# lxd99/TPNet

Measured on AMD Instinct MI355X. Metric: temporal edges/sec (proj-update + pairwise readout), higher is better.
Workload: dtype f32; 1 GPU; C2: Wikipedia-shape d=128 B=1000, L=3, synthetic S(8227,1000,E,span) stream of 2399000 edges, decoder-level unit (2 readouts + update per edge); batch=1000, dim=128, num_layer=3, nodes=9228, parallelism=single GPU

## Files before the change

tpnet_amd/csrc/api.hip:

```cpp
#include "tpnet_common.h"

#include <cstring>

namespace tpnet {
thread_local int g_last_hip_error = 0;

int check_state(const tpnet_state* st) {
    if (!st || !st->p0 || !st->q || !st->meta || !st->err) return TPNET_ERR_BAD_ARG;
    if (st->N < 1 || st->d < 1 || st->L < 1 || st->L > TPNET_MAX_LAYERS) return TPNET_ERR_BAD_ARG;
    if (st->N >= (1ll << 31)) return TPNET_ERR_BAD_ARG;
    return TPNET_OK;
}

template <class F> static int64_t most_that_fit(int64_t hi, F fits) {
    int64_t lo = 0;
    while (hi - lo > 1) {
        const int64_t mid = (lo + hi) / 2;
        if (fits(mid)) lo = mid; else hi = mid;
    }
    return lo;
}

static int64_t max_chunk(size_t ws_bytes, int64_t E, int64_t batch) {
    const int64_t hard = ((int64_t)1 << 30) / batch * batch;
// ... 123 lines not shown
};

static int run_stream_windowed(const StreamCall& c, int64_t chunk, int Kmax, size_t region) {
    const tpnet_state& st = c.st;
    const int64_t E = c.E, batch = c.batch;
    hipStream_t s = c.s;
    uint32_t lid = c.launch_id_base;
    const bool have_readout = c.out_pos || c.out_neg;
    char* const arena = reinterpret_cast<char*>((reinterpret_cast<size_t>(c.ws) + 255) / 256 * 256);
    const int64_t n_chunks = (E + chunk - 1) / chunk;
    float* const shared_log = region ? reinterpret_cast<float*>(arena + (size_t)n_chunks * region) : nullptr;
    PlanReplay tag(c, n_chunks == 1 || region, 1, true, window_batches_for(((E < chunk ? E : chunk) + batch - 1) / batch, Kmax),
                   c.flags & ~(uint32_t)TPNET_FLAG_SCHED_WINDOWED, have_readout, chunk, region);
    bool all_kept = true;
    for (int64_t c0 = 0, ci = 0; c0 < E; c0 += chunk, ++lid, ++ci) {
        const int64_t Ec = (E - c0 < chunk) ? (E - c0) : chunk;
        const int64_t nb = (Ec + batch - 1) / batch;
        const int K = window_batches_for(nb, Kmax);
        WPlan p{};
        int rc = region ? wplan_carve(arena + (size_t)ci * region, region, Ec, batch, st.N, st.d, st.L, K, &p, shared_log)
                        : wplan_carve(c.ws, c.ws_bytes, Ec, batch, st.N, st.d, st.L, K, &p);
        if (rc) return rc;
        const WPlanner planner = choose_wplanner(st, &p, Ec, batch, K, c.flags);
        all_kept &= planner.replayable;
        const StreamArgs a = c.args_at(c0);
        const WPlanArgs pa{a.src, a.dst, a.neg, a.t, Ec, batch, c.now_time, c0 > 0 ? c.t + c0 - 1 : nullptr, c.lambda, have_readout,
                           tag.replay};
        rc = planner.build(st, p, pa, s);
        if (rc) return rc;
        const int64_t nw = (Ec + p.Ew - 1) / p.Ew;
        const int64_t nsteps = nw + (have_readout ? st.L : st.L - 1);
        const bool timed = c.timer && c.timer->begin(s);
        for (int64_t j = 0; j < nsteps; ++j) {
            rc = launch_wstep(st, a, p, j, Ec, batch, c.lambda, c.flags, s);
            if (rc) return rc;
        }
        if (timed) c.timer->end(s, nsteps, Ec);
        rc = planner.writeback(st, p, Ec, batch, lid, s, -1);
        if (rc) return rc;
    }
    tag.commit(all_kept);
    return TPNET_OK;
}

static int run_stream_impl(const StreamCall& c) {
    const tpnet_state& st = c.st;
    const int64_t E = c.E, batch = c.batch;
    const double lambda = c.lambda;
    const uint32_t flags = c.flags;
    hipStream_t s = c.s;
    if (E == 0) return TPNET_OK;
    int Kw = 0;
    size_t region = 0;
    const int64_t wchunk = window_chunk(st, c.ws_bytes, E, batch, flags, &Kw, c.tag ? &region : nullptr);
    if (wchunk > 0) return run_stream_windowed(c, wchunk, Kw, region);
    const int64_t chunk = max_chunk(c.ws_bytes, E, batch);
    PlanReplay tag(c, chunk >= E, 2, false, 0, flags, c.out_pos != nullptr, chunk, 0);
    if (chunk < 1) return TPNET_ERR_WORKSPACE;
    uint32_t lid = c.launch_id_base;
    for (int64_t c0 = 0; c0 < E; c0 += chunk) {
        const int64_t Ec = (E - c0 < chunk) ? (E - c0) : chunk;
        Plan p{};
        int rc = plan_carve(c.ws, c.ws_bytes, Ec, batch, &p);
        if (rc) return rc;
        static const int fuse_env = TPNET_DEV_INT(FUSE, -1);
        static const int role_mask = TPNET_DEV_INT(ROLE_MASK, 3);
        const bool fuse = c.out_pos && p.fuse_src && role_mask == 3 &&
                          !(flags & (TPNET_FLAG_EAGER_DECAY | TPNET_FLAG_SEQUENTIAL)) &&
                          (fuse_env >= 0 ? fuse_env == 1 : batch > 1024);
        const StreamArgs a = c.args_at(c0);
        if (!tag.replay) {
            rc = plan_build(st, p, a.src, a.dst, a.t, Ec, batch, c.now_time, c0 > 0 ? c.t + c0 - 1 : nullptr, lambda,
// ... 408 lines not shown
```

tpnet_amd/csrc/plan.hip:

```cpp
#include "tpnet_common.h"

#include <cstdlib>
#include <cstring>
#include <rocprim/block/block_radix_sort.hpp>
#include <rocprim/device/device_radix_sort.hpp>
#include <rocprim/device/device_segmented_radix_sort.hpp>
#include <rocprim/iterator/counting_iterator.hpp>
#include <rocprim/iterator/transform_iterator.hpp>

#ifdef TPNET_STAMPS
#define PSTAMP(slot)                                                                          \
    do {                                                                                      \
        if (dbg && blockIdx.x == 0 && threadIdx.x == 0) {                                     \
            dbg[(slot) * 2 + 0] = __builtin_amdgcn_s_memtime();                               \
            dbg[(slot) * 2 + 1] = __builtin_amdgcn_s_memrealtime();                           \
        }                                                                                     \
    } while (0)
#else
#define PSTAMP(slot) do { } while (0)
#endif

namespace tpnet {

static constexpr uint32_t HEAVY_THRESHOLD = 8u;
// ... 802 lines not shown
                           node_bits, lambda, thr, fuse, st.err);
    TPNET_HIP_TRY(hipGetLastError());
    return TPNET_OK;
}


int wplan_window_batches(int64_t batch, int d, int L) {
    static const char* env = TPNET_DEV_STR(WINDOW);
    (void)L;
    if (d % 4 != 0 || d < 4 || batch < 1) return 0;
    if (batch > 4096) return 0;
    int64_t K = 24576 / batch;
    if (env) K = atoi(env);
    if (K > WIN_MAX_BATCHES) K = WIN_MAX_BATCHES;
    return K >= 2 ? (int)K : 0;
}

int window_batches_for(int64_t nb, int Kmax) {
    static const int fixed = TPNET_DEV_INT(WINDOW_FIXED, 0);
    if (fixed > 0) return fixed < Kmax ? fixed : Kmax;
    static const int num = TPNET_DEV_INT(WINDOW_SQ, 5);
    int K = 2;
    while (K < Kmax && (int64_t)K * K < (int64_t)num * nb) ++K;
    const int64_t nw0 = (nb + K - 1) / K;
    return (int)((nb + nw0 - 1) / nw0);
}

WPlanner choose_wplanner(const tpnet_state& st, const WPlan* p, int64_t Ec, int64_t batch, int K, uint32_t flags) {
    static const int no3 = TPNET_DEV_INT(NO_PLAN3, 0);
    static const int max3 = TPNET_DEV_INT(PLAN3_MAX_BATCHES, 1 << 30);
    const bool small = batch <= PLAN_ONE_MAX;
    if (!(flags & (TPNET_FLAG_PLAN_SORTED | TPNET_FLAG_PLAN_HASHED)) &&
        (p ? wplan_dense_applies(st, *p, Ec, batch, K) : small && wplan_dense_eligible(st.N, st.d, st.L, batch)))
        return {wplan_dense_build, wplan_dense_writeback, true, 256};
    if (!(flags & TPNET_FLAG_PLAN_SORTED) &&
        (p ? !no3 && (Ec + batch - 1) / batch <= max3 && wplan3_applies(st, Ec, batch, K) : small))
        return {wplan3_build, wplan3_writeback, true, WIN_MAX_WINDOWS};
    return {wplan_build, launch_wwriteback, false, 0};
}

bool wplan_medium_chains(int d) {
    static const int off = TPNET_DEV_INT(NO_MEDIUM, 0);
    if (off || d % 4 != 0) return false;
    const Geom g = pick_geom(d);
    return g.w == 4 && d == g.lpp * g.vpl * 4;
}

uint32_t wplan_heavy_threshold(int K, int64_t batch, int d) {
    static const int env = TPNET_DEV_INT(WIN_HEAVY, 0);
    if (env > 0) return (uint32_t)env;
    if (wplan_medium_chains(d)) return 128u;
    const int64_t t = (int64_t)K * batch * d / 24576;
    return (uint32_t)(t < 16 ? 16 : (t > 96 ? 96 : t));
}

int64_t wplan_max_chunk_edges(int64_t batch, int d, int L) {
    static const char* env = TPNET_DEV_STR(WIN_CHUNK_MB);
    const int64_t log_cap = (env ? (int64_t)atoi(env) : 16384) << 20;
    int64_t e = log_cap / (2 * (int64_t)L * d * 4);
    const int64_t hard = (int64_t)(WREF_SLOT_MASK >> 1);
    if (e > hard) e = hard;
    if (e > 65535 * batch) e = 65535 * batch;
    e = e / batch * batch;
    return e < batch ? batch : e;
}

static size_t wplan_extra_bytes(int64_t Ec, int64_t batch, int64_t N, int d, int L, int K) {
    const size_t nc = 2 * (size_t)Ec;
    (void)K;
    const size_t nw = (size_t)((Ec + batch - 1) / batch);
    size_t tot = 0;
// ... 445 lines not shown
```

tpnet_amd/csrc/tpnet_common.h:

```cpp
#pragma once
#include <hip/hip_runtime.h>
#include <stdint.h>
#include <stdlib.h>
#include <new>
#include "../../include/tpnet_hip.h"
#include "tpnet_dev.h"
#include "event_set.hpp"

#ifdef TPNET_DEV
static inline int tpnet_dev_env_int(const char* name, int dflt) { const char* v = getenv(name); return v ? atoi(v) : dflt; }
#define TPNET_DEV_INT(NAME, DFLT) tpnet_dev_env_int("TPNET_DEV_" #NAME, (DFLT))
#define TPNET_DEV_STR(NAME) getenv("TPNET_DEV_" #NAME)
#else
#define TPNET_DEV_INT(NAME, DFLT) (DFLT)
#define TPNET_DEV_STR(NAME) ((const char*)nullptr)
#endif

namespace tpnet {

struct NodeMeta {
    uint32_t ver;
    uint32_t pad0;
    double tref[2];
    uint64_t pad1;
// ... 240 lines not shown
                float* shared_log = nullptr, bool shard = false);
size_t wplan_bytes_shard(int64_t max_edges, int64_t batch, int64_t N, int d, int L);
size_t wplan_log_bytes(int64_t max_edges, int d, int L);
struct WPlanArgs {
    const int64_t *src, *dst, *neg;
    const double* t;
    int64_t Ec, batch;
    double now_time;
    const double* t_prev_dev;
    double lambda;
    bool want_readout;
    bool replay;
    int64_t own = -1;
    uint32_t* status = nullptr;
};
int wplan_build(const tpnet_state& st, const WPlan& p, const WPlanArgs& a, hipStream_t s);
int wplan3_build(const tpnet_state& st, const WPlan& p, const WPlanArgs& a, hipStream_t s);
int wplan_dense_build(const tpnet_state& st, const WPlan& p, const WPlanArgs& a, hipStream_t s);
int launch_wwriteback(const tpnet_state& st, const WPlan& p, int64_t Ec, int64_t batch, uint32_t launch_id, hipStream_t s, int64_t own = -1);
int wplan3_writeback(const tpnet_state& st, const WPlan& p, int64_t Ec, int64_t batch, uint32_t launch_id, hipStream_t s, int64_t own = -1);
int wplan_dense_writeback(const tpnet_state& st, const WPlan& p, int64_t Ec, int64_t batch, uint32_t launch_id, hipStream_t s, int64_t own = -1);
bool wplan3_applies(const tpnet_state& st, int64_t Ec, int64_t batch, int K);
size_t wplan3_table_bytes(int64_t Ec, int64_t batch);
size_t wplan3_blk_bytes(int64_t Ec, int64_t batch);
bool wplan_dense_eligible(int64_t N, int d, int L, int64_t batch);
size_t wplan_dense_bytes(int64_t Ec, int64_t batch, int64_t N, int d, int L);
bool wplan_dense_applies(const tpnet_state& st, const WPlan& p, int64_t Ec, int64_t batch, int K);
bool wplan_dense_applies_shard(const tpnet_state& st, const WPlan& p, int64_t Ec, int64_t batch, int K);

struct WPlanner {
    decltype(&wplan_build) build;
    decltype(&launch_wwriteback) writeback;
    bool replayable;
    int max_windows;
};
WPlanner choose_wplanner(const tpnet_state& st, const WPlan* p, int64_t Ec, int64_t batch, int K, uint32_t flags);
uint32_t wplan_heavy_threshold(int K, int64_t batch, int d);
bool wplan_medium_chains(int d);
int launch_wstep(const tpnet_state& st, const StreamArgs& a, const WPlan& p, int64_t j, int64_t Ec, int64_t batch,
                 double lambda, uint32_t flags, hipStream_t s);
int check_state(const tpnet_state* st);

extern thread_local int g_last_hip_error;
#define TPNET_HIP_TRY(expr)                                   \
    do {                                                      \
        hipError_t _e = (expr);                               \
        if (_e != hipSuccess) {                               \
            tpnet::g_last_hip_error = (int)_e;                \
            return TPNET_ERR_HIP;                             \
        }                                                     \
    } while (0)
#define TPNET_CATCH_BAD_ALLOC \
    catch (const std::bad_alloc&) { tpnet::g_last_hip_error = (int)hipErrorOutOfMemory; return TPNET_ERR_HIP; }

}
```

tpnet_amd/csrc/wshard.hip:

```cpp
#include "wplan_dense.hpp"

#include <rocprim/device/device_radix_sort.hpp>
#include <rocprim/device/device_scan.hpp>
#include <rocprim/iterator/counting_iterator.hpp>
#include <rocprim/iterator/transform_iterator.hpp>

#include <dlfcn.h>
#include <cstring>
#include <memory>
#include <vector>

namespace tpnet {

struct WsRccl {
    int (*send)(const void*, size_t, int, int, void*, hipStream_t) = nullptr;
    int (*recv)(void*, size_t, int, int, void*, hipStream_t) = nullptr;
    int (*group_start)() = nullptr;
    int (*group_end)() = nullptr;
};
bool rows_rccl_api(WsRccl* out);

static constexpr int WS_MAXG = 64;
static constexpr int kWsFloat32 = 7;

// ... 555 lines not shown
    if (phases & WS_PH_EXCHANGE) {
        WsRccl api;
        if (!comm || !rows_rccl_api(&api)) return TPNET_ERR_BAD_ARG;
        const size_t d = (size_t)w->st.d, Ld = (size_t)w->st.L * d;
        float* halo_p0 = w->st.p0 + (size_t)w->n_owned * d;
        float* halo_q = w->st.q + (size_t)w->n_owned * Ld;
        int bad = api.group_start();
        for (int r = 0; r < G; ++r) {
            if (r == me) continue;
            if (mine) {
                bad |= api.send(w->send_p0, (size_t)mine * d, kWsFloat32, r, comm, s);
                bad |= api.send(w->send_q, (size_t)mine * Ld, kWsFloat32, r, comm, s);
            }
            if (w->chunk_cnt[r]) {
                bad |= api.recv(halo_p0 + (size_t)w->hstart[r] * d, (size_t)w->chunk_cnt[r] * d, kWsFloat32, r, comm, s);
                bad |= api.recv(halo_q + (size_t)w->hstart[r] * Ld, (size_t)w->chunk_cnt[r] * Ld, kWsFloat32, r, comm, s);
            }
        }
        bad |= api.group_end();
        if (bad) return TPNET_ERR_HIP;
    }
    return TPNET_OK;
}

int tpnet_wshard_step(tpnet_wshard* w, void* comm, int64_t j, uint32_t phases, float* out_pos, float* out_neg, void* stream) {
    if (!w || j < 0 || j >= w->nsteps) return TPNET_ERR_BAD_ARG;
    hipStream_t s = (hipStream_t)stream;
    const int G = w->G, me = w->me, d = w->st.d, L = w->st.L;
    if (phases & WS_PH_LAUNCH) {
        StreamArgs a = w->a;
        a.out_pos = out_pos;
        a.out_neg = out_neg;
        if ((out_pos || out_neg) != w->have_readout) return TPNET_ERR_BAD_ARG;
        int rc = launch_wstep(w->st, a, w->p, j, w->E, w->batch, w->lambda, w->flags, s);
        if (rc) return rc;
    }
    if (G == 1) return TPNET_OK;
    const int64_t ns = w->send_base[j + 1] - w->send_base[j], nr = w->recv_base[j + 1] - w->recv_base[j];
    if ((phases & WS_PH_PACK) && ns > 0) {
        if (!w->sendbuf) return TPNET_ERR_BAD_ARG;
        int g = (int)((ns + 15) / 16);
        if (g > 4096) g = 4096;
        hipLaunchKernelGGL((k_ws_copy<true>), dim3(g), dim3(256), 0, s, w->ent[1] + w->send_base[j], (uint32_t)ns, w->p.log, w->sendbuf, L, d);
    }
    if ((phases & WS_PH_EXCHANGE) && (ns > 0 || nr > 0)) {
        WsRccl api;
        if (!comm || !rows_rccl_api(&api)) return TPNET_ERR_BAD_ARG;
        int bad = api.group_start();
        size_t so = 0, ro = 0;
        for (int r = 0; r < G; ++r) {
            const size_t cs = (size_t)w->send_cnt[(size_t)j * G + r], cr = (size_t)w->recv_cnt[(size_t)j * G + r];
            if (r != me && cs) bad |= api.send(w->sendbuf + so * d, cs * d, kWsFloat32, r, comm, s);
            if (r != me && cr) bad |= api.recv(w->recvbuf + ro * d, cr * d, kWsFloat32, r, comm, s);
            so += cs;
            ro += cr;
        }
        bad |= api.group_end();
        if (bad) return TPNET_ERR_HIP;
    }
    if ((phases & WS_PH_UNPACK) && nr > 0) {
        if (!w->recvbuf) return TPNET_ERR_BAD_ARG;
        int g = (int)((nr + 15) / 16);
        if (g > 4096) g = 4096;
        hipLaunchKernelGGL((k_ws_copy<false>), dim3(g), dim3(256), 0, s, w->ent[0] + w->recv_base[j], (uint32_t)nr, w->p.log, w->recvbuf, L, d);
    }
    TPNET_HIP_TRY(hipGetLastError());
    return TPNET_OK;
// ... 57 lines not shown
```

tpnet_amd/csrc/wstep.hip:

```cpp
#include "readout.hpp"

namespace tpnet {

static constexpr int WB = 256;
#ifndef TPNET_WPIPE_MINW
#define TPNET_WPIPE_MINW 4
#endif
constexpr int wpipe_min_waves(int lpp, int vpl, int l, bool full) {
    return (lpp <= 32 && vpl == 1) ? TPNET_WPIPE_MINW
         : (lpp == 32 && vpl == 2) ? ((full && l <= 3) ? 3 : 2)
         : (lpp == 64 && vpl == 1) ? (full ? 3 : 2)
         : 2;
}

__device__ __forceinline__ float pow_rep(float g, int n) {
    float r = 1.0f;
    for (int z = 0; z < n; ++z) r *= g;
    return r;
}

__device__ __forceinline__ const float* partner_row(const tpnet_state& S, const WPlan& P, int layer, int32_t pv,
                                                    uint32_t ref, float g, float& gp) {
    const int d = S.d, L = S.L;
    if (layer == 1) {
        gp = 1.0f;
        return S.p0 + (int64_t)pv * d;
    }
    gp = pow_rep(g, layer - 1);
    if (ref & WREF_TABLE) return S.q + (((int64_t)(ref & 1u) * S.N + pv) * L + (layer - 2)) * (int64_t)d;
    return P.log + ((int64_t)(ref & WREF_SLOT_MASK) * L + (layer - 2)) * (int64_t)d;
}

__device__ __forceinline__ const float* chain_start(const tpnet_state& S, const WPlan& P, const Chain& c, int layer,
                                                    float& g0) {
    const int d = S.d, L = S.L;
    g0 = pow_rep(c.g_first, layer);
    if (c.prev_ref & WREF_TABLE)
        return S.q + (((int64_t)(c.prev_ref & 1u) * S.N + c.target) * L + (layer - 1)) * (int64_t)d;
    return P.log + ((int64_t)(c.prev_ref & WREF_SLOT_MASK) * L + (layer - 1)) * (int64_t)d;
}

template <int LPP, int VPL, bool FULL>
__device__ __forceinline__ void chain_light(const tpnet_state& S, const WPlan& P, Chain c, bool valid, int layer,
                                            double lambda, int gl, unsigned long long* dbg) {
    (void)dbg;
    STAMP(5);
    constexpr int W = 4, F = VPL * W, U = (F == 4) ? 8 : 4;
    const int d = S.d, L = S.L;
    const int nvec = d / W;
    if (!valid) { c.cnt = 0; c.target = 0; c.j0 = 0; c.prev_ref = WREF_TABLE; c.g_first = 1.0f; }
    float g0;
    const float* qold = chain_start(S, P, c, layer, g0);
    const bool from_table = (c.prev_ref & WREF_TABLE) != 0;
    const int32_t* __restrict__ s_partner = P.base.s_partner;
    const float* __restrict__ s_coef = P.base.s_coef;

    for (int c0 = 0; c0 < (FULL ? 1 : nvec); c0 += LPP * VPL) {
        float acc[F], sblk[F], srun[F];
#pragma unroll
        for (int j = 0; j < VPL; ++j) {
            const int vi = c0 + j * LPP + gl;
            ldv_maybe<W, FULL>(qold, vi, valid && vi < nvec, &acc[j * W]);
        }
#pragma unroll
        for (int x = 0; x < F; ++x) { sblk[x] = 0.0f; srun[x] = 0.0f; }
        bool firstblk = false;
        float cur_dec = 1.0f;
        int32_t nx_pv = 0;
        float nx_w = 0.0f, nx_glog = 1.0f, nx_decr = 1.0f;
        uint32_t nx_ref = 0u;
        auto fetch_meta = [&](uint32_t r0) {
            const uint32_t jm = c.j0 + r0 + (uint32_t)gl;
            const bool mine = r0 + (uint32_t)gl < c.cnt;
            nx_pv = mine ? s_partner[jm] : 0;
            nx_w = mine ? s_coef[jm] : 0.0f;
            nx_ref = mine ? P.s_ref[jm] : 0u;
            nx_glog = mine ? P.s_g[jm] : 1.0f;
            nx_decr = mine ? P.s_dec[jm] : 1.0f;
        };
        fetch_meta(0u);
        for (uint32_t r0 = 0; __any(r0 < c.cnt); r0 += LPP) {
            const int32_t my_pv = nx_pv;
            const float my_w = nx_w;
            const uint32_t my_ref = nx_ref;
            const float my_glog = nx_glog;
            const float my_dec = pow_rep(nx_decr, layer);
// ... 39 lines not shown
                        }
                        if (fl & WREF_BLK_TAIL) {
#pragma unroll
                            for (int x = 0; x < F; ++x) srun[x] = firstblk ? sblk[x] : srun[x] + sblk[x];
                            firstblk = false;
                        }
                        if (fl & WREF_RUN_TAIL) {
#pragma unroll
                            for (int x = 0; x < F; ++x) {
                                acc[x] *= cur_dec;
                                acc[x] = acc[x] + srun[x];
                            }
                            float* lrow = P.log + ((int64_t)pos * L + (layer - 1)) * (int64_t)d;
#pragma unroll
                            for (int j = 0; j < VPL; ++j) {
                                const int vi = c0 + j * LPP + gl;
                                if (FULL || vi < nvec) stv<W>(lrow, vi, &acc[j * W]);
                            }
                        }
                    }
                }
            };
            if (__any(n_here > 0u)) issue(0u, rA);
            for (uint32_t k0 = 0; __any(k0 < n_here); k0 += 2 * US) {
                const bool more1 = __any(k0 + US < n_here);
                if (more1) issue(k0 + US, rB);
                consume(k0, rA);
                if (more1) {
                    if (__any(k0 + 2 * US < n_here)) issue(k0 + 2 * US, rA);
                    consume(k0 + US, rB);
                }
            }
        }
    }
    STAMP(6);
}

struct HRec {
    uint32_t row;
    float w, gp;
};
static_assert(sizeof(HRec) == 12, "HRec must be 12 bytes");

__device__ __forceinline__ uint32_t partner_row_index(const tpnet_state& S, int layer, int32_t pv, uint32_t ref, float g, float& gp,
                                                      bool& in_log) {
    const int L = S.L;
    in_log = false;
    if (layer == 1) {
        gp = 1.0f;
        return (uint32_t)pv;
    }
    gp = pow_rep(g, layer - 1);
    if (ref & WREF_TABLE) return (uint32_t)((((int64_t)(ref & 1u) * S.N + pv) * L) + (layer - 2));
    in_log = true;
    return (uint32_t)((int64_t)(ref & WREF_SLOT_MASK) * L + (layer - 2));
}

template <int LPH>
struct HeavyCfg {
    static constexpr int G = WB / LPH;
    static constexpr int PW = LPH * 4;
    static constexpr int TSEG = 128 * (8 * 4 + PW + 2) / (8 * 3 + PW + 2);
    static constexpr int HT = (TSEG + G - 1) / G < 4 ? (TSEG + G - 1) / G : 4;
    static constexpr int O_START = 0, O_END = 64, O_DECP = 128 , O_TOFF = 192 ,
                         O_RLIST = 260 , O_NRUN = 324, O_RTOFF = 328 , O_RSLOT = 396 ,
                         O_RSUM = 460 , O_REC = O_RSUM + 64 * PW ,
                         O_PART = O_REC + TSEG * WIN_BLOCK * 3 , O_TPOS = O_PART + TSEG * PW ,
                         O_TN = O_TPOS + TSEG , WORDS = O_TN + TSEG;
};

template <int LPH>
__device__ __forceinline__ void chain_heavy(const tpnet_state& S, const WPlan& P, const Chain c, int part, int layer,
                                            double lambda, uint32_t b0 ,
                                            uint32_t* __restrict__ lds_u, unsigned long long* dbg) {
    (void)dbg;
    STAMP(0);
    using H = HeavyCfg<LPH>;
    constexpr int G = H::G, PW = H::PW, TSEG = H::TSEG, HT = H::HT;
    const int tid = threadIdx.x, g = tid / LPH, gl = tid % LPH;
    const int d = S.d, L = S.L;
    const int nvec = d / 4;
    const int vi = part * LPH + gl;
    const bool vok = vi < nvec;
    uint32_t* run_start = lds_u + H::O_START;
    uint32_t* run_end = lds_u + H::O_END;
    float* r_decp = reinterpret_cast<float*>(lds_u + H::O_DECP);
    uint32_t* task_off = lds_u + H::O_TOFF;
    uint32_t* rlist = lds_u + H::O_RLIST;
    uint32_t* nrun_p = lds_u + H::O_NRUN;
    uint32_t* r_toff = lds_u + H::O_RTOFF;
    uint32_t* r_slot = lds_u + H::O_RSLOT;
    float* r_sum = reinterpret_cast<float*>(lds_u + H::O_RSUM);
    HRec* rec = reinterpret_cast<HRec*>(lds_u + H::O_REC);
    float* lds_part = reinterpret_cast<float*>(lds_u + H::O_PART);
    uint32_t* t_pos = lds_u + H::O_TPOS;
    uint32_t* t_n = lds_u + H::O_TN;

    __syncthreads();
    if (tid < 64) { run_start[tid] = 0xFFFFFFFFu; run_end[tid] = 0u; r_decp[tid] = 1.0f; }
    __syncthreads();
    float* dec_bw = r_sum;
    for (uint32_t p0 = 0; p0 < c.cnt; p0 += 8 * WB) {
        uint32_t ref[8], bcq[8];
        float dec[8];
#pragma unroll
        for (int q = 0; q < 8; ++q) {
            const uint32_t p = p0 + (uint32_t)(q * WB + tid);
            const bool in = p < c.cnt;
            ref[q] = in ? P.s_ref[c.j0 + p] : 0u;
            dec[q] = in ? P.s_dec[c.j0 + p] : 1.0f;
            bcq[q] = in ? (uint32_t)P.s_bc[c.j0 + p] : b0;
        }
#pragma unroll
        for (int q = 0; q < 8; ++q) {
            const uint32_t p = p0 + (uint32_t)(q * WB + tid);
            const uint32_t bw = (bcq[q] - b0) & 63u;
            if (ref[q] & WREF_RUN_HEAD) { run_start[bw] = p; dec_bw[bw] = dec[q]; }
            if (ref[q] & WREF_RUN_TAIL) run_end[bw] = p;
        }
    }
    __syncthreads();
    if (tid < 64) {
        const uint32_t st = run_start[tid];
        const bool has = st != 0xFFFFFFFFu;
        const uint32_t nt = has ? (run_end[tid] - st + WIN_BLOCK) / WIN_BLOCK : 0u;
        uint32_t inc = nt;
#pragma unroll
        for (int o = 1; o < 64; o <<= 1) {
            const uint32_t v = (uint32_t)__shfl_up((int)inc, o, 64);
// ... 157 lines not shown
                for (int q = 0; q < 4; ++q) {
                    const uint32_t rr = r0 + q;
                    if (rr < last) {
#pragma unroll
                        for (int x = 0; x < 4; ++x) {
                            acc[x] *= dec[q];
                            acc[x] = acc[x] + rs[q][x];
                        }
                        float* rs_ = r_sum + (size_t)rr * PW + gl * 4;
#pragma unroll
                        for (int x = 0; x < 4; ++x) rs_[x] = acc[x];
                    }
                }
            }
            if (tid == 0) nrun_p[1] = last;
        }
        __syncthreads();
        {
            const uint32_t lastb_ = nrun_p[1];
            for (uint32_t rr = next_run_all + (uint32_t)g; rr < lastb_; rr += G) {
                float v[4];
                const float* rs_ = r_sum + (size_t)rr * PW + gl * 4;
#pragma unroll
                for (int x = 0; x < 4; ++x) v[x] = rs_[x];
                if (vok) {
                    float* lrow = P.log + ((int64_t)r_slot[rr] * L + (layer - 1)) * (int64_t)d;
                    stv<4>(lrow, vi, v);
                }
            }
            next_run_all = lastb_;
        }
        if (tid < 64) next_run = last;
        __syncthreads();
    }
    STAMP(4);
#ifdef TPNET_STAMPS
    if (dbg && (threadIdx.x & 63) == 0) {
        const size_t wv = ((size_t)blockIdx.x * (blockDim.x >> 6) + (threadIdx.x >> 6));
        if (wv < 4000) dbg[(wv * 8 + 7) * 2 + 0] = c.cnt;
    }
#endif
}

template <int LPP, int VPL, int LWORDS>
struct MedCfg {
    static constexpr int GPB = WB / LPP;
    static constexpr int PG = GPB * 16 <= WB ? 16 : WB / GPB;
    static constexpr int SEGP = GPB * PG;
    static constexpr int RW = LPP * VPL * 4;
    static constexpr int O_ROW = 0, O_W = 2 * SEGP, O_GP = 3 * SEGP, O_FL = 4 * SEGP, O_DEC = 5 * SEGP, O_BLK = 6 * SEGP,
                         O_BFL = 7 * SEGP, BCAP_ = (LWORDS - 7 * SEGP - (GPB + 1) - 16 - 4) / (RW + 3),
                         BCAP = BCAP_ > SEGP ? SEGP : BCAP_, O_BDEC = O_BFL + BCAP, O_BSLOT = O_BDEC + BCAP,
                         O_OWN = O_BSLOT + BCAP, O_MISC = O_OWN + GPB + 1, O_SUM = (O_MISC + 16 + 3) / 4 * 4,
                         WORDS = O_SUM + BCAP * RW;
    static_assert(WORDS <= LWORDS, "chain_medium: LDS layout");
    static_assert(BCAP >= 8, "chain_medium: LDS for at least 8 block sums");
};

template <int LPP, int VPL, int LWORDS>
__device__ __forceinline__ void chain_medium(const tpnet_state& S, const WPlan& P, const Chain c, int layer,
                                             uint32_t* __restrict__ lds_u) {
    using M = MedCfg<LPP, VPL, LWORDS>;
    constexpr int W = 4, F = VPL * W, U = (F == 4) ? 8 : 4;
    constexpr int GPB = M::GPB, SEGP = M::SEGP, BCAP = M::BCAP, RW = M::RW;
    static_assert(SEGP <= WB, "a thread per position");
    const int tid = threadIdx.x, g = tid / LPP, gl = tid % LPP;
    const int d = S.d, L = S.L;
    const float** p_row = reinterpret_cast<const float**>(lds_u + M::O_ROW);
    float* p_w = reinterpret_cast<float*>(lds_u + M::O_W);
    float* p_gp = reinterpret_cast<float*>(lds_u + M::O_GP);
    uint32_t* p_fl = lds_u + M::O_FL;
    float* p_dec = reinterpret_cast<float*>(lds_u + M::O_DEC);
    uint32_t* p_blk = lds_u + M::O_BLK;
    uint32_t* b_fl = lds_u + M::O_BFL;
    float* b_dec = reinterpret_cast<float*>(lds_u + M::O_BDEC);
    uint32_t* b_slot = lds_u + M::O_BSLOT;
    uint32_t* own = lds_u + M::O_OWN;
    uint32_t* misc = lds_u + M::O_MISC;
    float* bsum = reinterpret_cast<float*>(lds_u + M::O_SUM);

    float g0;
    const float* qold = chain_start(S, P, c, layer, g0);
    const bool from_table = (c.prev_ref & WREF_TABLE) != 0;
    float acc[F], srun[F];
#pragma unroll
    for (int j = 0; j < VPL; ++j) ldv<W>(g == 0 ? qold : S.p0, j * LPP + gl, &acc[j * W]);
#pragma unroll
    for (int x = 0; x < F; ++x) srun[x] = 0.0f;
    bool firstblk = false;
    float cur_dec = 1.0f;

    for (uint32_t s0 = 0; s0 < c.cnt;) {
        __syncthreads();
        const uint32_t left = c.cnt - s0 < (uint32_t)SEGP ? c.cnt - s0 : (uint32_t)SEGP;
        const uint32_t pg = (left + GPB - 1) / GPB < 2u ? 2u : (left + GPB - 1) / GPB;
        const uint32_t pos = s0 + (uint32_t)tid;
        const bool in = tid < SEGP && pos < c.cnt;
        const uint32_t jm = c.j0 + (in ? pos : 0u);
        const int32_t pv = in ? P.base.s_partner[jm] : 0;
        const float wgt = in ? P.base.s_coef[jm] : 0.0f;
        const uint32_t ref = in ? P.s_ref[jm] : 0u;
        const float glog = in ? P.s_g[jm] : 1.0f;
        const float decr = in ? P.s_dec[jm] : 1.0f;
        if (tid <= GPB) own[tid] = SEGP;
        const bool head = in && (ref & WREF_BLK_HEAD) != 0;
        const unsigned long long hm = __ballot(head);
        const int lane = tid & 63, wave = tid >> 6;
        if (lane == 0 && wave < 4) misc[2 + wave] = (uint32_t)__popcll(hm);
        __syncthreads();
        uint32_t blk = (uint32_t)__popcll(hm & ((2ull << lane) - 1ull)) - 1u;
        for (int wv = 0; wv < wave && wv < 4; ++wv) blk += misc[2 + wv];
        const bool keep = in && blk < (uint32_t)BCAP;
        if (tid < SEGP) {
            float gp;
            const float* row = partner_row(S, P, layer, pv, ref, glog, gp);
            p_row[tid] = row;
// ... 73 lines not shown
                    sb[j * W] = v4.x; sb[j * W + 1] = v4.y; sb[j * W + 2] = v4.z; sb[j * W + 3] = v4.w;
                }
                if (bf & 1u) { firstblk = true; cur_dec = b_dec[b]; }
#pragma unroll
                for (int x = 0; x < F; ++x) srun[x] = firstblk ? sb[x] : srun[x] + sb[x];
                firstblk = false;
                if (bf & 2u) {
#pragma unroll
                    for (int x = 0; x < F; ++x) {
                        acc[x] *= cur_dec;
                        acc[x] = acc[x] + srun[x];
                    }
#pragma unroll
                    for (int j = 0; j < VPL; ++j)
                        slot[j * LPP + gl] = make_float4(acc[j * W], acc[j * W + 1], acc[j * W + 2], acc[j * W + 3]);
                }
            }
        }
        __syncthreads();
        for (uint32_t b = (uint32_t)g; b < nblk; b += GPB) {
            if (b_fl[b] & 2u) {
                const float4* slot = reinterpret_cast<const float4*>(bsum + (size_t)b * RW);
                float* lrow = P.log + ((int64_t)b_slot[b] * L + (layer - 1)) * (int64_t)d;
#pragma unroll
                for (int j = 0; j < VPL; ++j) {
                    const float4 v4 = slot[j * LPP + gl];
                    const float v[4] = {v4.x, v4.y, v4.z, v4.w};
                    stv<W>(lrow, j * LPP + gl, v);
                }
            }
        }
        s0 += npos;
    }
}

constexpr int heavy_lph(int lpp, int vpl) { return lpp * vpl <= 32 ? 4 : (lpp * vpl <= 64 ? 8 : 16); }

struct WStep {
    int64_t w_upd[TPNET_MAX_LAYERS];
    int64_t w_read;
    uint32_t seg[2 * TPNET_MAX_LAYERS + 3];
    int32_t CP;
    int32_t dbg_layer;
    int32_t dbg_skip;
    uint32_t n_active;
    uint32_t hub_ext;
    uint32_t hub_blocks;
    uint32_t med;
};

__device__ __forceinline__ uint32_t big_chains(const WStep& st, const WinDesc& wd, uint32_t n_hub) {
    const uint32_t n = st.med == 3u ? wd.n_med : st.med == 2u ? wd.n_ext : st.med == 1u ? wd.n_ext1 : 0u;
    return n > n_hub ? n : n_hub;
}

__device__ __forceinline__ uint32_t hub_chains(const WStep& st, const WinDesc& wd) {
    if (st.hub_ext == 2 && wd.n_ext * (uint32_t)st.CP <= st.hub_blocks) return wd.n_ext;
    if (st.hub_ext >= 1 && wd.n_ext1 * (uint32_t)st.CP <= st.hub_blocks) return wd.n_ext1;
    return wd.n_heavy;
}

template <int LPP, int VPL, int L, bool FULL, bool RS, bool SHARD = false>
__global__ __launch_bounds__(WB, wpipe_min_waves(LPP, VPL, L, FULL)) void k_wpipe(tpnet_state S, WPlan P, StreamArgs a, WStep st, int64_t Ec, int64_t B,
                                              double lambda, uint32_t flags) {
    constexpr int W = 4;
    constexpr int LPH = heavy_lph(LPP, VPL);
    constexpr int RLPP = RS ? 16 : LPP, RVPL = RS ? 2 : VPL;
    static_assert(!RS || (LPP == 32 && VPL == 1), "readout split: chains on 32 x 1");
    using C = GramCfg<RLPP, L>;
    constexpr bool LR = false;
    constexpr int RWORDS = (RLPP < 16) ? C::NG * (WB / RLPP) : 1;
    constexpr int LWORDS = HeavyCfg<LPH>::WORDS > RWORDS ? HeavyCfg<LPH>::WORDS : RWORDS;
    constexpr int SL = 2 * L;
    __shared__ __attribute__((aligned(16))) uint32_t lds_u[LWORDS];
    const int gl = threadIdx.x % LPP;
    const int g = threadIdx.x / LPP;
    constexpr int GPB = WB / LPP;
    const uint32_t bx = blockIdx.x;
    int sidx = 0;
    uint32_t seg_lo = 0, seg_hi = st.seg[1];
    int64_t w = st.w_upd[0];
#pragma unroll
// ... 72 lines not shown
                const float gs_e = P.e_g[(int64_t)which[s] * Ec + e];
                const uint32_t ref = idok ? ref_e : WREF_TABLE;
                const float gs = idok ? gs_e : 1.0f;
                const float* qb = (ref & WREF_TABLE) ? S.q + ((int64_t)(ref & 1u) * S.N + ids[s]) * ((int64_t)L * d)
                                                     : P.log + (int64_t)(ref & WREF_SLOT_MASK) * ((int64_t)L * d);
                rowp[s * NR] = S.p0 + ids[s] * (int64_t)d;
                rs[s * NR] = 1.0f;
                float gg = 1.0f;
#pragma unroll
                for (int i = 1; i <= L; ++i) {
                    gg *= gs;
                    rowp[s * NR + i] = qb + (int64_t)(i - 1) * d;
                    rs[s * NR + i] = gg;
                }
            }
            if (packed)
                gram_rows<RLPP, RVPL, W, L, FULL, true, LR>(rowp, rs, d, valid, idok, do_scale, out, rgl, stage);
            else
                gram_rows<RLPP, RVPL, W, L, FULL, false, LR>(rowp, rs, d, valid, idok, do_scale, out, rgl, stage);
        }
        BEND();
        return;
    }
    const WinDesc wd = P.wdesc[w];
    unsigned long long* dbg = (st.dbg_layer == layer) ? P.base.dbg : nullptr;
    (void)dbg;
    if (sidx < L) {
#ifdef TPNET_DEV
        if (st.dbg_skip & 1) return;
#endif
        const Chain* __restrict__ heavy = P.chains + wd.start;
        const uint32_t units = hub_chains(st, wd) * (uint32_t)st.CP;
        for (uint32_t h = rb; h < units; h += nblk)
            chain_heavy<LPH>(S, P, heavy[h / (uint32_t)st.CP], (int)(h % (uint32_t)st.CP), layer, lambda,
                             (uint32_t)(w * P.K), lds_u, dbg);
        BEND();
        return;
    }
    if (sidx < SL) {
        if constexpr (FULL) {
            const uint32_t n_hub = hub_chains(st, wd);
            const uint32_t n_big = big_chains(st, wd, n_hub);
            const Chain* __restrict__ list = P.chains + wd.start;
            for (uint32_t m = n_hub + rb; m < n_big; m += nblk) chain_medium<LPP, VPL, LWORDS>(S, P, list[m], layer, lds_u);
        }
        BEND();
        return;
    }
#ifdef TPNET_DEV
    if (st.dbg_skip & 2) return;
#endif
    const uint32_t n_hub = big_chains(st, wd, hub_chains(st, wd));
    const Chain* __restrict__ small = P.chains + wd.start + n_hub;
    const int64_t n_small = (int64_t)wd.n_chains - (int64_t)n_hub;
    for (int64_t base = (int64_t)rb * GPB; base < n_small; base += (int64_t)nblk * GPB) {
        const int64_t idx = base + g;
        const bool valid = idx < n_small;
        const Chain c = small[valid ? idx : 0];
        chain_light<LPP, VPL, FULL>(S, P, c, valid, layer, lambda, gl, dbg);
    }
    BEND();
}

static constexpr int WBS = 256;
__global__ __launch_bounds__(WB) void k_wwriteback(tpnet_state S, WPlan P, int64_t nc, uint32_t bid) {
    const int per = S.L * S.d;
    NodeMeta* meta = reinterpret_cast<NodeMeta*>(S.meta);
    __shared__ uint32_t n_list;
    __shared__ uint32_t l_pos[WBS];
    __shared__ int32_t l_node[WBS];
    __shared__ int32_t l_copy[WBS];
    for (int64_t j0 = (int64_t)blockIdx.x * WBS; j0 < nc; j0 += (int64_t)gridDim.x * WBS) {
        __syncthreads();
        if (threadIdx.x == 0) n_list = 0;
        __syncthreads();
        const int64_t j = j0 + threadIdx.x;
        if (threadIdx.x < WBS && j < nc && (P.s_ref[j] & WREF_LAST_RUN)) {
            const int32_t u = P.base.s_target[j];
            const int c = (int)(meta[u].ver & 1u);
            const uint32_t k = atomicAdd(&n_list, 1u);
            l_pos[k] = (uint32_t)j;
            l_node[k] = u;
            l_copy[k] = c;
        }
        __syncthreads();
        const uint32_t n = n_list;
        if ((per & 3) == 0) {
            const uint32_t pv = (uint32_t)per / 4;
            const uint32_t tot = n * pv;
            for (uint32_t x0 = threadIdx.x; x0 < tot; x0 += 4 * WB) {
                const uint32_t xa = x0, xb = x0 + WB, xc = x0 + 2 * WB, xd = x0 + 3 * WB;
                const uint32_t ka = xa / pv, kb = (xb < tot ? xb : xa) / pv, kc = (xc < tot ? xc : xa) / pv, kd = (xd < tot ? xd : xa) / pv;
// ... 2 lines not shown
                const float4 va = reinterpret_cast<const float4*>(P.log + (int64_t)l_pos[ka] * per)[oa];
                const float4 vb = reinterpret_cast<const float4*>(P.log + (int64_t)l_pos[kb] * per)[ob];
                const float4 vc = reinterpret_cast<const float4*>(P.log + (int64_t)l_pos[kc] * per)[oc];
                const float4 vd = reinterpret_cast<const float4*>(P.log + (int64_t)l_pos[kd] * per)[od];
                reinterpret_cast<float4*>(S.q + ((int64_t)(l_copy[ka] ^ 1) * S.N + l_node[ka]) * (int64_t)per)[oa] = va;
                if (xb < tot) reinterpret_cast<float4*>(S.q + ((int64_t)(l_copy[kb] ^ 1) * S.N + l_node[kb]) * (int64_t)per)[ob] = vb;
                if (xc < tot) reinterpret_cast<float4*>(S.q + ((int64_t)(l_copy[kc] ^ 1) * S.N + l_node[kc]) * (int64_t)per)[oc] = vc;
                if (xd < tot) reinterpret_cast<float4*>(S.q + ((int64_t)(l_copy[kd] ^ 1) * S.N + l_node[kd]) * (int64_t)per)[od] = vd;
            }
        } else {
            for (uint32_t x = threadIdx.x; x < n * (uint32_t)per; x += WB) {
                const uint32_t k = x / (uint32_t)per, o = x - k * (uint32_t)per;
                S.q[((int64_t)(l_copy[k] ^ 1) * S.N + l_node[k]) * (int64_t)per + o] = P.log[(int64_t)l_pos[k] * per + o];
            }
        }
        if (threadIdx.x < n) {
            const uint32_t k = threadIdx.x;
            publish_meta(meta + l_node[k], l_copy[k] ^ 1, P.base.desc[P.s_bc[l_pos[k]]].t_last, bid);
        }
    }
}

int launch_wwriteback(const tpnet_state& st, const WPlan& p, int64_t Ec, int64_t, uint32_t launch_id, hipStream_t s, int64_t) {
    const int64_t nc = 2 * Ec;
    int64_t grid = (nc + WBS - 1) / WBS;
    if (grid > 16384) grid = 16384;
    if (grid < 1) grid = 1;
    hipLaunchKernelGGL(k_wwriteback, dim3((unsigned)grid), dim3(WB), 0, s, st, p, nc, launch_id);
    TPNET_HIP_TRY(hipGetLastError());
    return TPNET_OK;
}

int launch_wstep(const tpnet_state& st, const StreamArgs& a, const WPlan& p, int64_t j, int64_t Ec, int64_t batch,
                 double lambda, uint32_t flags, hipStream_t s) {
    if ((reinterpret_cast<uintptr_t>(a.out_pos) | reinterpret_cast<uintptr_t>(a.out_neg)) & 15) return TPNET_ERR_BAD_ARG;
    if (st.d % 4 != 0) return TPNET_ERR_BAD_ARG;
    const int L = st.L;
    const int64_t nw = (Ec + p.Ew - 1) / p.Ew;
    static const int hb_env = TPNET_DEV_INT(WIN_HB, 0);
    static const int stamp_layer = TPNET_DEV_INT(STAMP_LAYER, 0);
    static const int geo_env = TPNET_DEV_INT(WIN_GEOM, 0);
    const Geom geo = pick_geom(st.d, geo_env == 1);
    const int lph = heavy_lph(geo.lpp, geo.vpl);
    const int GPB = WB / geo.lpp;
    static const int rs_env = TPNET_DEV_INT(WIN_RSPLIT, 1);
    const bool rsplit = rs_env == 1 && geo.lpp == 32 && geo.vpl == 1 && st.d / 4 > 16;
    WStep ws;
    ws.CP = (st.d / 4 + lph - 1) / lph;
    static const int stamp_step = TPNET_DEV_INT(STAMP_STEP, -1);
    ws.dbg_layer = (stamp_layer == -1 && stamp_step >= 0 && j != stamp_step) ? 0 : stamp_layer;
    static const int skip_env = TPNET_DEV_INT(WIN_SKIP, 0);
    ws.dbg_skip = skip_env;
    const bool have_readout = a.out_pos || a.out_neg;
    auto win_edges = [&](int64_t w) { const int64_t e0 = w * p.Ew; return (Ec - e0 < p.Ew) ? Ec - e0 : p.Ew; };
    uint32_t nb = 0;
    for (int i = 0; i < TPNET_MAX_LAYERS; ++i) ws.w_upd[i] = -1;
    static const int ext_env = TPNET_DEV_INT(WIN_HUB_EXT, 2);
    int n_upd = 0;
    for (int i = 0; i < L; ++i) n_upd += (j - i >= 0 && j - i < nw) ? 1 : 0;
    const bool reads = have_readout && j - L >= 0 && j - L < nw;
    const bool med_on = wplan_medium_chains(st.d);
    ws.hub_ext = (!med_on && ext_env >= 1 && n_upd == 1 && (!reads || p.K >= 14)) ? 2u : 0u;
    if (!med_on && ext_env >= 2 && n_upd == 2 && !reads && p.K >= 14) ws.hub_ext = 1u;
    const uint32_t hub_blocks = ws.hub_ext ? (uint32_t)(hb_env > 0 ? hb_env : 384) * (uint32_t)L / (uint32_t)n_upd
                                           : (uint32_t)(hb_env > 0 ? hb_env : 384);
    ws.hub_blocks = hub_blocks;
    for (int i = 0; i < L; ++i) {
// ... 9 lines not shown
    static const int med_part = TPNET_DEV_INT(WIN_MED_PART, 3);
    ws.med = wplan_medium_chains(st.d) ? (uint32_t)((n_upd == L && reads) ? med_full : med_part) : 0u;
    for (int i = 0; i < L; ++i) {
        ws.seg[L + i] = nb;
        if (ws.med && ws.w_upd[i] >= 0) nb += (uint32_t)(mb_env > 0 ? mb_env : 384);
    }
    ws.seg[2 * L] = nb;
    {
        uint32_t nact = 0, per = 0;
        for (int i = 0; i < L; ++i) {
            if (ws.w_upd[i] >= 0) {
                ++nact;
                static const int lb_env = TPNET_DEV_INT(WIN_LB, 0);
                const uint32_t g_ = (uint32_t)grid_for(2 * win_edges(ws.w_upd[i]) / 3 + 1, GPB, lb_env > 0 ? lb_env : 768);
                per = g_ > per ? g_ : per;
            }
        }
        ws.n_active = nact ? nact : 1;
        nb += nact * per;
    }
    ws.seg[2 * L + 1] = nb;
    ws.w_read = -1;
    {
        const int64_t w = j - L;
        if (have_readout && w >= 0 && w < nw) {
            ws.w_read = w;
            const int64_t npairs = (a.out_pos ? win_edges(w) : 0) + (a.out_neg ? win_edges(w) : 0);
            nb += (uint32_t)grid_for(npairs, rsplit ? WB / 16 : GPB, 256 * 8);
        }
    }
    ws.seg[2 * L + 2] = nb;
    if (nb == 0) return TPNET_OK;
    const bool shard = a.own_mod == 0;
    TPNET_DISPATCH_G(geo, ({
        if constexpr (W == 4) {
            if constexpr (LPP == 32 && VPL == 1) {
                if (rsplit && shard)
                    hipLaunchKernelGGL((k_wpipe<LPP, VPL, L, FULL, true, true>), dim3(nb), dim3(WB), 0, s, st, p, a, ws, Ec, batch, lambda, flags);
                else if (rsplit)
                    hipLaunchKernelGGL((k_wpipe<LPP, VPL, L, FULL, true>), dim3(nb), dim3(WB), 0, s, st, p, a, ws, Ec, batch, lambda, flags);
                else if (shard)
                    hipLaunchKernelGGL((k_wpipe<LPP, VPL, L, FULL, false, true>), dim3(nb), dim3(WB), 0, s, st, p, a, ws, Ec, batch, lambda, flags);
                else
                    hipLaunchKernelGGL((k_wpipe<LPP, VPL, L, FULL, false>), dim3(nb), dim3(WB), 0, s, st, p, a, ws, Ec, batch, lambda, flags);
            } else {
                if (shard)
                    hipLaunchKernelGGL((k_wpipe<LPP, VPL, L, FULL, false, true>), dim3(nb), dim3(WB), 0, s, st, p, a, ws, Ec, batch, lambda, flags);
                else
                    hipLaunchKernelGGL((k_wpipe<LPP, VPL, L, FULL, false>), dim3(nb), dim3(WB), 0, s, st, p, a, ws, Ec, batch, lambda, flags);
            }
        } else {
            return TPNET_ERR_BAD_ARG;
        }
    }));
    TPNET_HIP_TRY(hipGetLastError());
    return TPNET_OK;
}

}
```

Before: 355.2 million edges/s.

## Fuse final-state writeback into windowed step kernels for replayable planners

The per-chunk writeback kernel, which copies each node's final projection rows into the double-buffered table and publishes node metadata, is folded into the chain update kernels (light, medium, heavy). When a chain's last run is processed, the accumulator is stored directly to the opposite table copy and the metadata is published at the last layer. This removes a separate launch and re-reading of the log, at the cost of extra per-chain branching, metadata loads and register pressure in the hot step kernels. It applies only to the dense and plan3 planners, not the sharded path.

Measured after the change: 348.2 million edges/s. 0.98x the previous value.

```diff
diff --git a/tpnet_amd/csrc/api.hip b/tpnet_amd/csrc/api.hip
--- a/tpnet_amd/csrc/api.hip
+++ b/tpnet_amd/csrc/api.hip
@@ -179,12 +179,14 @@
         const int64_t nsteps = nw + (have_readout ? st.L : st.L - 1);
         const bool timed = c.timer && c.timer->begin(s);
         for (int64_t j = 0; j < nsteps; ++j) {
-            rc = launch_wstep(st, a, p, j, Ec, batch, c.lambda, c.flags, s);
+            rc = launch_wstep(st, a, p, j, Ec, batch, c.lambda, c.flags, lid, planner.steps_write_back, s);
             if (rc) return rc;
         }
         if (timed) c.timer->end(s, nsteps, Ec);
-        rc = planner.writeback(st, p, Ec, batch, lid, s, -1);
-        if (rc) return rc;
+        if (!planner.steps_write_back) {
+            rc = planner.writeback(st, p, Ec, batch, lid, s, -1);
+            if (rc) return rc;
+        }
     }
     tag.commit(all_kept);
     return TPNET_OK;
diff --git a/tpnet_amd/csrc/plan.hip b/tpnet_amd/csrc/plan.hip
--- a/tpnet_amd/csrc/plan.hip
+++ b/tpnet_amd/csrc/plan.hip
@@ -858,11 +858,11 @@
     const bool small = batch <= PLAN_ONE_MAX;
     if (!(flags & (TPNET_FLAG_PLAN_SORTED | TPNET_FLAG_PLAN_HASHED)) &&
         (p ? wplan_dense_applies(st, *p, Ec, batch, K) : small && wplan_dense_eligible(st.N, st.d, st.L, batch)))
-        return {wplan_dense_build, wplan_dense_writeback, true, 256};
+        return {wplan_dense_build, wplan_dense_writeback, true, true, 256};
     if (!(flags & TPNET_FLAG_PLAN_SORTED) &&
         (p ? !no3 && (Ec + batch - 1) / batch <= max3 && wplan3_applies(st, Ec, batch, K) : small))
-        return {wplan3_build, wplan3_writeback, true, WIN_MAX_WINDOWS};
-    return {wplan_build, launch_wwriteback, false, 0};
+        return {wplan3_build, wplan3_writeback, true, true, WIN_MAX_WINDOWS};
+    return {wplan_build, launch_wwriteback, false, false, 0};
 }
 
 bool wplan_medium_chains(int d) {
diff --git a/tpnet_amd/csrc/tpnet_common.h b/tpnet_amd/csrc/tpnet_common.h
--- a/tpnet_amd/csrc/tpnet_common.h
+++ b/tpnet_amd/csrc/tpnet_common.h
@@ -296,13 +296,14 @@
     decltype(&wplan_build) build;
     decltype(&launch_wwriteback) writeback;
     bool replayable;
+    bool steps_write_back;
     int max_windows;
 };
 WPlanner choose_wplanner(const tpnet_state& st, const WPlan* p, int64_t Ec, int64_t batch, int K, uint32_t flags);
 uint32_t wplan_heavy_threshold(int K, int64_t batch, int d);
 bool wplan_medium_chains(int d);
 int launch_wstep(const tpnet_state& st, const StreamArgs& a, const WPlan& p, int64_t j, int64_t Ec, int64_t batch,
-                 double lambda, uint32_t flags, hipStream_t s);
+                 double lambda, uint32_t flags, uint32_t launch_id, bool write_back, hipStream_t s);
 int check_state(const tpnet_state* st);
 
 extern thread_local int g_last_hip_error;
diff --git a/tpnet_amd/csrc/wshard.hip b/tpnet_amd/csrc/wshard.hip
--- a/tpnet_amd/csrc/wshard.hip
+++ b/tpnet_amd/csrc/wshard.hip
@@ -611,7 +611,7 @@
         a.out_pos = out_pos;
         a.out_neg = out_neg;
         if ((out_pos || out_neg) != w->have_readout) return TPNET_ERR_BAD_ARG;
-        int rc = launch_wstep(w->st, a, w->p, j, w->E, w->batch, w->lambda, w->flags, s);
+        int rc = launch_wstep(w->st, a, w->p, j, w->E, w->batch, w->lambda, w->flags, 0u, false, s);
         if (rc) return rc;
     }
     if (G == 1) return TPNET_OK;
diff --git a/tpnet_amd/csrc/wstep.hip b/tpnet_amd/csrc/wstep.hip
--- a/tpnet_amd/csrc/wstep.hip
+++ b/tpnet_amd/csrc/wstep.hip
@@ -35,14 +35,68 @@
                                                     float& g0) {
     const int d = S.d, L = S.L;
     g0 = pow_rep(c.g_first, layer);
-    if (c.prev_ref & WREF_TABLE)
-        return S.q + (((int64_t)(c.prev_ref & 1u) * S.N + c.target) * L + (layer - 1)) * (int64_t)d;
-    return P.log + ((int64_t)(c.prev_ref & WREF_SLOT_MASK) * L + (layer - 1)) * (int64_t)d;
-}
-
-template <int LPP, int VPL, bool FULL>
+    const int64_t lo = (int64_t)(layer - 1) * d, per = (int64_t)L * d;
+    if (c.prev_ref & WREF_TABLE) return (S.q + lo) + ((int64_t)(c.prev_ref & 1u) * S.N + c.target) * per;
+    return (P.log + lo) + (int64_t)(c.prev_ref & WREF_SLOT_MASK) * per;
+}
+
+struct WStep {
+    int64_t w_upd[TPNET_MAX_LAYERS];
+    int64_t w_read;
+    uint32_t seg[2 * TPNET_MAX_LAYERS + 3];
+    int32_t CP;
+    int32_t dbg_layer;
+    int32_t dbg_skip;
+    uint32_t n_active;
+    uint32_t hub_ext;
+    uint32_t hub_blocks;
+    uint32_t med;
+    uint32_t wb;
+    uint32_t bid;
+};
+
+struct WPipeArgs {
+    tpnet_state S;
+    WPlan P;
+    StreamArgs a;
+    WStep st;
+    int64_t Ec, B;
+    double lambda;
+    uint32_t flags;
+};
+typedef const WPipeArgs __attribute__((address_space(4)))* WPipeArgsPtr;
+__device__ __forceinline__ WPipeArgsPtr wpipe_args_now() {
+    WPipeArgsPtr p = (WPipeArgsPtr)__builtin_amdgcn_kernarg_segment_ptr();
+    asm volatile("" : "+s"(p));
+    return p;
+}
+
+typedef uint32_t WBack;
+template <bool ON>
+__device__ __forceinline__ WBack wback_of(const tpnet_state& S, const WPlan& P, const Chain& c, bool valid, uint32_t wb, uint32_t bid) {
+    if constexpr (ON) {
+        if (wb) {
+            const uint32_t jl = c.cnt ? c.j0 + c.cnt - 1u : 0u;
+            const uint32_t ref = P.s_ref[jl];
+            const uint32_t bc = (uint32_t)P.s_bc[jl];
+            const uint32_t ver = reinterpret_cast<const NodeMeta*>(S.meta)[c.target].ver;
+            uint32_t cur = ver & 1u;
+            if ((ver >> 1) == bid) cur ^= 1u;
+            return (valid && c.cnt && (ref & WREF_LAST_RUN)) ? (1u + (cur ^ 1u)) | (bc << 2) : 0u;
+        }
+    }
+    return 0u;
+}
+__device__ __forceinline__ float* wback_row(const tpnet_state& S, WBack b, int32_t target, int layer) {
+    return S.q + (((int64_t)((b & 3u) - 1u) * S.N + target) * S.L + (layer - 1)) * (int64_t)S.d;
+}
+__device__ __forceinline__ void wback_publish(const tpnet_state& S, const WPlan& P, WBack b, int32_t target, uint32_t bid) {
+    publish_meta(reinterpret_cast<NodeMeta*>(S.meta) + target, (int)((b & 3u) - 1u), P.base.desc[b >> 2].t_last, bid);
+}
+
+template <int LPP, int VPL, bool FULL, bool WBK>
 __device__ __forceinline__ void chain_light(const tpnet_state& S, const WPlan& P, Chain c, bool valid, int layer,
-                                            double lambda, int gl, unsigned long long* dbg) {
+                                            double lambda, int gl, uint32_t* __restrict__ lds_u, unsigned long long* dbg) {
     (void)dbg;
     STAMP(5);
     constexpr int W = 4, F = VPL * W, U = (F == 4) ? 8 : 4;
@@ -52,6 +106,7 @@
     float g0;
     const float* qold = chain_start(S, P, c, layer, g0);
     const bool from_table = (c.prev_ref & WREF_TABLE) != 0;
+    if constexpr (WBK) lds_u[threadIdx.x] = (uint32_t)c.target;
     const int32_t* __restrict__ s_partner = P.base.s_partner;
     const float* __restrict__ s_coef = P.base.s_coef;
 
@@ -157,6 +212,28 @@
                 }
             }
         }
+        if constexpr (WBK) {
+            const WPipeArgsPtr ka = wpipe_args_now();
+            if (ka->st.wb) {
+                const uint32_t jl = c.cnt ? c.j0 + c.cnt - 1u : 0u;
+                const int32_t target = (int32_t)lds_u[threadIdx.x];
+                const uint32_t wb_ref = ka->P.s_ref[jl];
+                const uint32_t wb_bc = (uint32_t)ka->P.s_bc[jl];
+                const uint32_t wb_ver = reinterpret_cast<const NodeMeta*>(ka->S.meta)[target].ver;
+                if (valid && c.cnt != 0u && (wb_ref & WREF_LAST_RUN)) {
+                    const uint32_t to = ((((wb_ver >> 1) == ka->st.bid) ? wb_ver ^ 1u : wb_ver) & 1u) ^ 1u;
+                    const int Lk = ka->S.L;
+                    float* trow = ka->S.q + (((int64_t)to * ka->S.N + target) * Lk + (layer - 1)) * (int64_t)ka->S.d;
+#pragma unroll
+                    for (int j = 0; j < VPL; ++j) {
+                        const int vi = c0 + j * LPP + gl;
+                        if (FULL || vi < nvec) stv<W>(trow, vi, &acc[j * W]);
+                    }
+                    if (layer == Lk && gl == 0 && c0 + LPP * VPL >= (FULL ? 1 : nvec))
+                        publish_meta(reinterpret_cast<NodeMeta*>(ka->S.meta) + target, (int)to, ka->P.base.desc[wb_bc].t_last, ka->st.bid);
+                }
+            }
+        }
     }
     STAMP(6);
 }
@@ -194,9 +271,9 @@
                          O_TN = O_TPOS + TSEG , WORDS = O_TN + TSEG;
 };
 
-template <int LPH>
+template <int LPH, bool WBK>
 __device__ __forceinline__ void chain_heavy(const tpnet_state& S, const WPlan& P, const Chain c, int part, int layer,
-                                            double lambda, uint32_t b0 ,
+                                            double lambda, uint32_t b0 , uint32_t wb, uint32_t bid,
                                             uint32_t* __restrict__ lds_u, unsigned long long* dbg) {
     (void)dbg;
     STAMP(0);
@@ -220,6 +297,7 @@
     float* lds_part = reinterpret_cast<float*>(lds_u + H::O_PART);
     uint32_t* t_pos = lds_u + H::O_TPOS;
     uint32_t* t_n = lds_u + H::O_TN;
+    const WBack wbk = wback_of<WBK>(S, P, c, true, wb, bid);
 
     __syncthreads();
     if (tid < 64) { run_start[tid] = 0xFFFFFFFFu; run_end[tid] = 0u; r_decp[tid] = 1.0f; }
@@ -443,6 +521,10 @@
         }
         if (tid < 64) next_run = last;
         __syncthreads();
+    }
+    if (WBK && wbk) {
+        if (g == 0 && vok) stv<4>(wback_row(S, wbk, c.target, layer), vi, acc);
+        if (layer == L && part == 0 && tid == 0) wback_publish(S, P, wbk, c.target, bid);
     }
     STAMP(4);
 #ifdef TPNET_STAMPS
@@ -468,9 +550,9 @@
     static_assert(BCAP >= 8, "chain_medium: LDS for at least 8 block sums");
 };
 
-template <int LPP, int VPL, int LWORDS>
-__device__ __forceinline__ void chain_medium(const tpnet_state& S, const WPlan& P, const Chain c, int layer,
-                                             uint32_t* __restrict__ lds_u) {
+template <int LPP, int VPL, int LWORDS, bool WBK>
+__device__ __forceinline__ void chain_medium(const tpnet_state& S, const WPlan& P, const Chain c, int layer, uint32_t wb,
+                                             uint32_t bid, uint32_t* __restrict__ lds_u) {
     using M = MedCfg<LPP, VPL, LWORDS>;
     constexpr int W = 4, F = VPL * W, U = (F == 4) ? 8 : 4;
     constexpr int GPB = M::GPB, SEGP = M::SEGP, BCAP = M::BCAP, RW = M::RW;
@@ -493,6 +575,7 @@
     float g0;
     const float* qold = chain_start(S, P, c, layer, g0);
     const bool from_table = (c.prev_ref & WREF_TABLE) != 0;
+    const WBack wbk = wback_of<WBK>(S, P, c, true, wb, bid);
     float acc[F], srun[F];
 #pragma unroll
     for (int j = 0; j < VPL; ++j) ldv<W>(g == 0 ? qold : S.p0, j * LPP + gl, &acc[j * W]);
@@ -632,22 +715,17 @@
         }
         s0 += npos;
     }
+    if (WBK && wbk) {
+        if (g == 0) {
+            float* trow = wback_row(S, wbk, c.target, layer);
+#pragma unroll
+            for (int j = 0; j < VPL; ++j) stv<W>(trow, j * LPP + gl, &acc[j * W]);
+        }
+        if (layer == L && tid == 0) wback_publish(S, P, wbk, c.target, bid);
+    }
 }
 
 constexpr int heavy_lph(int lpp, int vpl) { return lpp * vpl <= 32 ? 4 : (lpp * vpl <= 64 ? 8 : 16); }
-
-struct WStep {
-    int64_t w_upd[TPNET_MAX_LAYERS];
-    int64_t w_read;
-    uint32_t seg[2 * TPNET_MAX_LAYERS + 3];
-    int32_t CP;
-    int32_t dbg_layer;
-    int32_t dbg_skip;
-    uint32_t n_active;
-    uint32_t hub_ext;
-    uint32_t hub_blocks;
-    uint32_t med;
-};
 
 __device__ __forceinline__ uint32_t big_chains(const WStep& st, const WinDesc& wd, uint32_t n_hub) {
     const uint32_t n = st.med == 3u ? wd.n_med : st.med == 2u ? wd.n_ext : st.med == 1u ? wd.n_ext1 : 0u;
@@ -786,8 +864,8 @@
         const Chain* __restrict__ heavy = P.chains + wd.start;
         const uint32_t units = hub_chains(st, wd) * (uint32_t)st.CP;
         for (uint32_t h = rb; h < units; h += nblk)
-            chain_heavy<LPH>(S, P, heavy[h / (uint32_t)st.CP], (int)(h % (uint32_t)st.CP), layer, lambda,
-                             (uint32_t)(w * P.K), lds_u, dbg);
+            chain_heavy<LPH, !SHARD>(S, P, heavy[h / (uint32_t)st.CP], (int)(h % (uint32_t)st.CP), layer, lambda,
+                                     (uint32_t)(w * P.K), st.wb, st.bid, lds_u, dbg);
         BEND();
         return;
     }
@@ -796,7 +874,7 @@
             const uint32_t n_hub = hub_chains(st, wd);
             const uint32_t n_big = big_chains(st, wd, n_hub);
             const Chain* __restrict__ list = P.chains + wd.start;
-            for (uint32_t m = n_hub + rb; m < n_big; m += nblk) chain_medium<LPP, VPL, LWORDS>(S, P, list[m], layer, lds_u);
+            for (uint32_t m = n_hub + rb; m < n_big; m += nblk) chain_medium<LPP, VPL, LWORDS, !SHARD>(S, P, list[m], layer, st.wb, st.bid, lds_u);
         }
         BEND();
         return;
@@ -811,7 +889,7 @@
         const int64_t idx = base + g;
         const bool valid = idx < n_small;
         const Chain c = small[valid ? idx : 0];
-        chain_light<LPP, VPL, FULL>(S, P, c, valid, layer, lambda, gl, dbg);
+        chain_light<LPP, VPL, FULL, !SHARD>(S, P, c, valid, layer, lambda, gl, lds_u, dbg);
     }
     BEND();
 }
@@ -880,7 +958,7 @@
 }
 
 int launch_wstep(const tpnet_state& st, const StreamArgs& a, const WPlan& p, int64_t j, int64_t Ec, int64_t batch,
-                 double lambda, uint32_t flags, hipStream_t s) {
+                 double lambda, uint32_t flags, uint32_t launch_id, bool write_back, hipStream_t s) {
     if ((reinterpret_cast<uintptr_t>(a.out_pos) | reinterpret_cast<uintptr_t>(a.out_neg)) & 15) return TPNET_ERR_BAD_ARG;
     if (st.d % 4 != 0) return TPNET_ERR_BAD_ARG;
     const int L = st.L;
@@ -956,6 +1034,9 @@
     ws.seg[2 * L + 2] = nb;
     if (nb == 0) return TPNET_OK;
     const bool shard = a.own_mod == 0;
+    if (shard && write_back) return TPNET_ERR_BAD_ARG;
+    ws.wb = write_back ? 1u : 0u;
+    ws.bid = launch_id;
     TPNET_DISPATCH_G(geo, ({
         if constexpr (W == 4) {
             if constexpr (LPP == 32 && VPL == 1) {
```
